# sony/timbre-trap

Measured on AMD Instinct MI355X. Metric: audio-seconds/s training throughput (9oct x 60bpo, 3s@22.05kHz), higher is better.
Workload: dtype bf16; 1 GPU; full train step (CQT x2 + AE fwd/bwd with consistency + 3 losses + clip + AdamW), model_complexity=2 latent=128, 64 clips x 3 s per GPU, under torch.autocast like reference experiments/train.py:415 (bf16 MFMA conv path of BASELINE config[2]; fp32 master weights, losses and optimizer); global_batch=64, parallelism=dp1

## Files before the change

### timbre-trap_amd/csrc/conv_edge_bf16.hip

```cpp
#include "bf16_common.h"
#include <type_traits>

namespace {

constexpr int ETH = 16, ETW = 64, ERW = ETW + 2, EROWS = ETH + 2;
constexpr int EPLANE = EROWS * ERW;
constexpr int PP = ETW + 8, PPLANE = EROWS * PP, PCOL0 = 3;
constexpr int NPARTW = 80;

__device__ __forceinline__ float gatef(float dy, float y) { return dy * elu_dout(y); }

struct ETile { int b, h0, t0; };
__device__ __forceinline__ ETile etile(int v, int tiles_h, int tiles_t, int ntiles) {
    int tile = xcd_order(v, ntiles);
    ETile r;
    r.t0 = (tile % tiles_t) * ETW; tile /= tiles_t;
    r.h0 = (tile % tiles_h) * ETH;
    r.b = tile / tiles_h;
    return r;
}

struct TileCtx { ETile tl; bool interior, interior_v; };
__device__ __forceinline__ TileCtx tile_ctx(int v, int tiles_h, int tiles_t, int ntiles, int H, int T) {
    TileCtx c;
// ... 428 lines not shown
        const ETile tl = etile(v, tiles_h, tiles_t, ntiles);
        __syncthreads();
        sx.store(xs, tid);
        __syncthreads();
        flush();
        if (v + gridDim.x < ntiles) sx.load(x, nullptr, tile_ctx(v + gridDim.x, tiles_h, tiles_t, ntiles, H, T), H, T, tid);
        PWin xw;
        xw.start(xs, r0, lane);
#pragma unroll
        for (int rr = 0; rr < ERPW; ++rr) {
            xw.advance(xs, r0 + rr, lane);
            if constexpr (NO == 2) {
                f32x2 a4[4] = {br, splat2(0.f), splat2(0.f), splat2(0.f)};
                static_for<0, 36>([&](auto ic) {
                    constexpr int ci = decltype(ic)::value / 9, k = decltype(ic)::value % 9;
                    a4[ci] = wr[ci * 9 + k] * xw.template tap<k, ci>() + a4[ci];
                });
                o[rr] = (a4[0] + a4[1]) + (a4[2] + a4[3]);
            } else {
                f32x2 a2[2] = {br, splat2(0.f)};
                static_for<0, 18>([&](auto ic) {
                    constexpr int p = decltype(ic)::value / 9, k = decltype(ic)::value % 9;
                    a2[p] = wr[p * 9 + k] * xw.template pair<k, p>() + a2[p];
                });
                const f32x2 a = a2[0] + a2[1];
                o[rr][0] = act_out(a[0] + a[1], ACT);
                o[rr][1] = 0.f;
            }
            asm volatile("" : "+v"(o[rr]));
            row_fence();
        }
        tp = tl;
    }
    flush();
}

template <bool VEC, int NO = 2, int ACT = TT_ACT_NONE>
__global__ __launch_bounds__(NT, 2) void k_cout_bwd(const e16* __restrict__ x, const float* __restrict__ dy, const float* __restrict__ w,
                                                  e16* __restrict__ dx, float* __restrict__ part, int H, int T, int tiles_h,
                                                  int tiles_t, int ntiles, float scale, const float* __restrict__ ysaved = nullptr) {
    constexpr int NW = NO * 36;
    __shared__ __attribute__((aligned(16))) float xs[4 * EPLANE + 4];
    __shared__ __attribute__((aligned(16))) float gs[NO * PPLANE];
    __shared__ float red[4 * (NW + NO)];
    const int tid = threadIdx.x, lane = tid & 63, wave = tid >> 6;
    float wa[NO * 9];
#pragma unroll
    for (int i = 0; i < NO * 9; ++i) wa[i] = scale * w[((i / 9) * 4 + (lane & 3)) * 9 + i % 9];
    f32x2 acc[NO == 2 ? 36 : 18], accb = splat2(0.f);
#pragma unroll
    for (int i = 0; i < (NO == 2 ? 36 : 18); ++i) acc[i] = splat2(0.f);
    StageCl4<false> sx;
    StagePlanar<NO, VEC, NO == 2 ? TT_ACT_NONE : ACT> sg;
    sx.init(T, tid); sg.init(H, T, tid);
    if (blockIdx.x < ntiles) {
        const TileCtx t0 = tile_ctx(blockIdx.x, tiles_h, tiles_t, ntiles, H, T);
        sx.load(x, nullptr, t0, H, T, tid); sg.load(dy, t0, H, T, tid, ysaved);
    }
    for (int v = blockIdx.x; v < ntiles; v += gridDim.x) {
        const ETile tl = etile(v, tiles_h, tiles_t, ntiles);
        __syncthreads();
        sx.store(xs, tid);
        sg.store(gs, tid);
        __syncthreads();
        if (v + gridDim.x < ntiles) {
            const TileCtx tn = tile_ctx(v + gridDim.x, tiles_h, tiles_t, ntiles, H, T);
            sx.load(x, nullptr, tn, H, T, tid); sg.load(dy, tn, H, T, tid, ysaved);
        }
        const int t = tl.t0 + lane, r0 = wave * ERPW;
        {
            PWin xw;
            xw.start(xs, r0, lane);
#pragma unroll
            for (int rr = 0; rr < ERPW; ++rr) {
                const int r = r0 + rr, ctr = (r + 1) * PP + lane + PCOL0 + 1;
                xw.advance(xs, r, lane);
                f32x2 g;
                if constexpr (NO == 2) {
                    g[0] = gs[ctr]; g[1] = gs[PPLANE + ctr];
                    accb += g;
                    static_for<0, 36>([&](auto ic) {
                        constexpr int i = decltype(ic)::value;
                        acc[i] = g * xw.template tap<i % 9, i / 9>() + acc[i];
                    });
                } else {
                    g = splat2(gs[ctr]);
                    accb[0] += g[0];
                    static_for<0, 18>([&](auto ic) {
                        constexpr int i = decltype(ic)::value;
                        acc[i] = g * xw.template pair<i % 9, i / 9>() + acc[i];
                    });
                }
                pin(acc); asm volatile("" : "+v"(accb));
                row_fence();
            }
        }
        f32x4 d[ERPW];
#pragma unroll
        for (int rr = 0; rr < ERPW; ++rr) d[rr] = f32x4{0.f, 0.f, 0.f, 0.f};
#pragma unroll
        for (int co = 0; co < NO; ++co) {
            WRow<1> gw[ERPW + 2];
#pragma unroll
            for (int i = 0; i < ERPW + 2; ++i) gw[i].load(gs + co * PPLANE, (r0 + i) * PP + lane + PCOL0);
            taps9<0>([&](auto kc) {
                constexpr int k = decltype(kc)::value;
#pragma unroll
                for (int rr = 0; rr < ERPW; ++rr) d[rr] = mfma441(wa[co * 9 + k], gw[rr + 2 - k / 3].template one<2 - k % 3>(0), d[rr]);
            });
            row_fence();
        }
#pragma unroll
        for (int rr = 0; rr < ERPW; ++rr) {
            const int h = tl.h0 + r0 + rr;
            e16x4 o;
            o[0] = (e16)d[rr][0]; o[1] = (e16)d[rr][1]; o[2] = (e16)d[rr][2]; o[3] = (e16)d[rr][3];
            if (t < T && h < H) *reinterpret_cast<e16x4*>(dx + (((long)tl.b * H + h) * T + t) * 4) = o;
        }
    }
    __syncthreads();
    float flat[NW + NO];
    if constexpr (NO == 2) {
#pragma unroll
        for (int i = 0; i < 36; ++i) { flat[i] = acc[i][0]; flat[36 + i] = acc[i][1]; }
        flat[72] = accb[0]; flat[73] = accb[1];
    } else {
#pragma unroll
        for (int i = 0; i < 18; ++i) { flat[(2 * (i / 9)) * 9 + i % 9] = acc[i][0]; flat[(2 * (i / 9) + 1) * 9 + i % 9] = acc[i][1]; }
        flat[36] = accb[0];
    }
    const float tot = wg_total<NW + NO>(flat, red, tid);
    if (tid < NW + NO) part[(long)blockIdx.x * NPARTW + tid] = tot;
}

__global__ __launch_bounds__(1024) void k_edge_reduce(const float* __restrict__ part, int nwg, float* __restrict__ dw, float* __restrict__ db,
                                                       int nb, float scale, int nw = 72) {
    __shared__ float red[16][64];
    const int el = threadIdx.x & 63, sl = threadIdx.x >> 6;
    const int e = blockIdx.x * 64 + el;
    float s = 0.f;
    if (e < nw + nb)
        for (int j = sl; j < nwg; j += 16) s += part[(long)j * NPARTW + e];
    red[sl][el] = s;
    __syncthreads();
    if (sl != 0 || e >= nw + nb) return;
    float sum = 0.f;
#pragma unroll
    for (int i = 0; i < 16; ++i) sum += red[i][el];
    if (e < nw) dw[e] += sum * scale; else db[e - nw] += sum * scale;
}

constexpr int EDGE_MAX_WG = 1024;

inline bool edge_ok(int B, int H, int T) { return B > 0 && H > 0 && T > 0 && (long)H * T * 4 < (1l << 31); }
inline void edge_tiles(int B, int H, int T, int& th, int& tt, int& n) { th = (H + ETH - 1) / ETH; tt = (T + ETW - 1) / ETW; n = B * th * tt; }
inline int edge_grid(int ntiles) { const int cap = 4 * tt_cus(); const int g = ntiles < cap ? ntiles : cap; return g < EDGE_MAX_WG ? g : EDGE_MAX_WG; }

}

extern "C" {

int64_t tt_edge16_scratch_bytes(void) { return (int64_t)EDGE_MAX_WG * NPARTW * 4; }

int tt_convin16_fwd(const float* x, const float* w, const float* b, void* y, int B, int H, int T, void* stream) {
    if (!x || !w || !b || !y || !edge_ok(B, H, T)) return TT_E_BADARG;
    int th, tt, n; edge_tiles(B, H, T, th, tt, n);
    if (T % 4 == 0) hipLaunchKernelGGL(k_cin_fwd<true>, dim3(edge_grid(n)), dim3(NT), 0, tt_stream(stream), x, w, b, (e16*)y, H, T, th, tt, n);
    else hipLaunchKernelGGL(k_cin_fwd<false>, dim3(edge_grid(n)), dim3(NT), 0, tt_stream(stream), x, w, b, (e16*)y, H, T, th, tt, n);
    TT_LAUNCH_CHECK();
    return 0;
}

int tt_convin16_bwd(const float* x, const void* y, const void* dy, const float* w, float* dx, float* dw, float* db, void* ws, int B,
                    int H, int T, void* stream) {
    if (!x || !dy || !w || !dw || !db || !ws || !edge_ok(B, H, T)) return TT_E_BADARG;
    int th, tt, n; edge_tiles(B, H, T, th, tt, n);
    const int grid = edge_grid(n);
    hipStream_t st = tt_stream(stream);
    const bool vec = T % 4 == 0;
#define CIN_BWD(DX_, V_, P_) hipLaunchKernelGGL((k_cin_bwd<DX_, V_, P_>), dim3(grid), dim3(NT), 0, st, x, (const e16*)y, (const e16*)dy, w, dx, (float*)ws, H, T, th, tt, n, tt_loss_unscale())
    if (y) {
        if (dx) { if (vec) CIN_BWD(true, true, false); else CIN_BWD(true, false, false); }
        else { if (vec) CIN_BWD(false, true, false); else CIN_BWD(false, false, false); }
    } else {
        if (dx) { if (vec) CIN_BWD(true, true, true); else CIN_BWD(true, false, true); }
        else { if (vec) CIN_BWD(false, true, true); else CIN_BWD(false, false, true); }
    }
#undef CIN_BWD
    TT_LAUNCH_CHECK();
    hipLaunchKernelGGL(k_edge_reduce, dim3(2), dim3(1024), 0, st, (const float*)ws, grid, dw, db, 4, tt_loss_unscale());
    TT_LAUNCH_CHECK();
    return 0;
}

int tt_convout16_fwd(const void* x, const float* w, const float* b, float* y, int B, int H, int T, void* stream) {
    if (!x || !w || !b || !y || !edge_ok(B, H, T)) return TT_E_BADARG;
    int th, tt, n; edge_tiles(B, H, T, th, tt, n);
    hipLaunchKernelGGL(k_cout_fwd, dim3(edge_grid(n)), dim3(NT), 0, tt_stream(stream), (const e16*)x, w, b, y, H, T, th, tt, n);
    TT_LAUNCH_CHECK();
    return 0;
}

int tt_convout16_bwd(const void* x, const float* dy, const float* w, void* dx, float* dw, float* db, void* ws, int B, int H, int T,
                     void* stream) {
    if (!x || !dy || !w || !dx || !dw || !db || !ws || !edge_ok(B, H, T)) return TT_E_BADARG;
    int th, tt, n; edge_tiles(B, H, T, th, tt, n);
    const int grid = edge_grid(n);
    hipStream_t st = tt_stream(stream);
    if (T % 4 == 0) hipLaunchKernelGGL(k_cout_bwd<true>, dim3(grid), dim3(NT), 0, st, (const e16*)x, dy, w, (e16*)dx, (float*)ws, H, T, th, tt, n, tt_loss_scale());
    else hipLaunchKernelGGL(k_cout_bwd<false>, dim3(grid), dim3(NT), 0, st, (const e16*)x, dy, w, (e16*)dx, (float*)ws, H, T, th, tt, n, tt_loss_scale());
    TT_LAUNCH_CHECK();
    hipLaunchKernelGGL(k_edge_reduce, dim3(2), dim3(1024), 0, st, (const float*)ws, grid, dw, db, 2, 1.f);
    TT_LAUNCH_CHECK();
    return 0;
}

int tt_convin16_1_fwd(const float* x, const float* w, const float* b, void* y, int B, int H, int T, void* stream) {
    if (!x || !w || !b || !y || !edge_ok(B, H, T)) return TT_E_BADARG;
    int th, tt, n; edge_tiles(B, H, T, th, tt, n);
    if (T % 4 == 0) hipLaunchKernelGGL((k_cin_fwd<true, 1>), dim3(edge_grid(n)), dim3(NT), 0, tt_stream(stream), x, w, b, (e16*)y, H, T, th, tt, n);
    else hipLaunchKernelGGL((k_cin_fwd<false, 1>), dim3(edge_grid(n)), dim3(NT), 0, tt_stream(stream), x, w, b, (e16*)y, H, T, th, tt, n);
    TT_LAUNCH_CHECK();
    return 0;
}

int tt_convin16_1_bwd(const float* x, const void* y, const void* dy, const float* w, float* dx, float* dw, float* db, void* ws, int B,
                      int H, int T, void* stream) {
    if (!x || !dy || !w || !dw || !db || !ws || !edge_ok(B, H, T)) return TT_E_BADARG;
    int th, tt, n; edge_tiles(B, H, T, th, tt, n);
    const int grid = edge_grid(n);
    hipStream_t st = tt_stream(stream);
    const bool vec = T % 4 == 0;
#define CIN1_BWD(DX_, V_, P_) hipLaunchKernelGGL((k_cin_bwd<DX_, V_, P_, 1>), dim3(grid), dim3(NT), 0, st, x, (const e16*)y, (const e16*)dy, w, dx, (float*)ws, H, T, th, tt, n, tt_loss_unscale())
    if (y) {
        if (dx) { if (vec) CIN1_BWD(true, true, false); else CIN1_BWD(true, false, false); }
        else { if (vec) CIN1_BWD(false, true, false); else CIN1_BWD(false, false, false); }
    } else {
        if (dx) { if (vec) CIN1_BWD(true, true, true); else CIN1_BWD(true, false, true); }
        else { if (vec) CIN1_BWD(false, true, true); else CIN1_BWD(false, false, true); }
    }
#undef CIN1_BWD
    TT_LAUNCH_CHECK();
    hipLaunchKernelGGL(k_edge_reduce, dim3(1), dim3(1024), 0, st, (const float*)ws, grid, dw, db, 4, tt_loss_unscale(), 36);
    TT_LAUNCH_CHECK();
    return 0;
}

int tt_convout16_1_fwd(const void* x, const float* w, const float* b, float* y, int B, int H, int T, int act, void* stream) {
    if (!x || !w || !b || !y || !edge_ok(B, H, T)) return TT_E_BADARG;
    int th, tt, n; edge_tiles(B, H, T, th, tt, n);
    hipStream_t st = tt_stream(stream);
    const dim3 grid(edge_grid(n));
    if (act == TT_ACT_NONE) hipLaunchKernelGGL((k_cout_fwd<1, TT_ACT_NONE>), grid, dim3(NT), 0, st, (const e16*)x, w, b, y, H, T, th, tt, n);
    else if (act == TT_ACT_RELU) hipLaunchKernelGGL((k_cout_fwd<1, TT_ACT_RELU>), grid, dim3(NT), 0, st, (const e16*)x, w, b, y, H, T, th, tt, n);
    else if (act == TT_ACT_SIGMOID) hipLaunchKernelGGL((k_cout_fwd<1, TT_ACT_SIGMOID>), grid, dim3(NT), 0, st, (const e16*)x, w, b, y, H, T, th, tt, n);
    else return TT_E_BADARG;
    TT_LAUNCH_CHECK();
    return 0;
}

int tt_convout16_1_bwd(const void* x, const float* y, const float* dy, const float* w, void* dx, float* dw, float* db, void* ws, int B, int H,
                       int T, int act, void* stream) {
    if (!x || !dy || !w || !dx || !dw || !db || !ws || !edge_ok(B, H, T)) return TT_E_BADARG;
    if ((act != TT_ACT_NONE && act != TT_ACT_RELU && act != TT_ACT_SIGMOID) || (act != TT_ACT_NONE && !y)) return TT_E_BADARG;
    int th, tt, n; edge_tiles(B, H, T, th, tt, n);
    const int grid = edge_grid(n);
    hipStream_t st = tt_stream(stream);
    const float s = tt_loss_scale();
#define COUT1_BWD(V_, A_) hipLaunchKernelGGL((k_cout_bwd<V_, 1, A_>), dim3(grid), dim3(NT), 0, st, (const e16*)x, dy, w, (e16*)dx, (float*)ws, H, T, th, tt, n, s, y)
    if (T % 4 == 0) {
        if (act == TT_ACT_NONE) COUT1_BWD(true, TT_ACT_NONE); else if (act == TT_ACT_RELU) COUT1_BWD(true, TT_ACT_RELU); else COUT1_BWD(true, TT_ACT_SIGMOID);
    } else {
        if (act == TT_ACT_NONE) COUT1_BWD(false, TT_ACT_NONE); else if (act == TT_ACT_RELU) COUT1_BWD(false, TT_ACT_RELU); else COUT1_BWD(false, TT_ACT_SIGMOID);
    }
#undef COUT1_BWD
    TT_LAUNCH_CHECK();
    hipLaunchKernelGGL(k_edge_reduce, dim3(1), dim3(1024), 0, st, (const float*)ws, grid, dw, db, 1, 1.f, 36);
    TT_LAUNCH_CHECK();
    return 0;
}

}
```

### timbre-trap_amd/timbre_trap/_hip.py

```python

import ctypes
import os
import subprocess
import sys

_HERE = os.path.dirname(os.path.abspath(__file__))
PKG_ROOT = os.path.dirname(_HERE)
REPO_ROOT = os.path.dirname(PKG_ROOT)
CSRC = os.path.join(PKG_ROOT, 'csrc')
LIB_PATH = os.path.join(PKG_ROOT, 'lib', 'libttrap_hip.so')
if os.environ.get('TTRAP_LIB'):
    LIB_PATH = os.path.join(PKG_ROOT, 'lib', os.environ['TTRAP_LIB'])
SOURCES = ['cqt.hip', 'cqt_generic.hip', 'conv_generic.hip', 'conv_mfma.hip', 'conv_small.hip', 'conv_wide_bf16.hip', 'conv_level_bf16.hip', 'conv_stride_bf16.hip',
           'latent_bf16.hip', 'conv_edge_bf16.hip', 'gemm.hip', 'losses.hip', 'magnitude.hip',
           'conv_wide_f16.hip', 'conv_level_f16.hip', 'conv_stride_f16.hip', 'latent_f16.hip', 'conv_edge_f16.hip',
           'conv_x3.hip',
           'sdr.hip',
           'mpe.hip',
           'resample.hip',
           'notes.hip',
           'pitch.hip',
           'film.hip',
           'mix.hip']

# ... 31 lines not shown
    'tt_conv2d_wgrad': (c_int, [P, P, P, P, I, I, I, I, I, I, I, I, I, I, I, I, I, L, L, L, L, P]),
    'tt_elu_bwd': (c_int, [P, P, P, L, P]),
    'tt_act_bwd': (c_int, [P, P, P, L, I, P]),
    'tt_cqt_forward_mag': (c_int, [ctypes.POINTER(CqtPlan), P, P, P, I, I, P]),
    'tt_magnitude': (c_int, [P, P, L, L, P]),
    'tt_decibels_scratch_bytes': (c_int64, [L]),
    'tt_decibels': (c_int, [P, P, L, L, I, P, P]),
    'tt_activations1_fwd': (c_int, [P, P, L, P]),
    'tt_activations1_bwd': (c_int, [P, P, P, L, P]),
    'tt_resblock_fwd': (c_int, [P, P, P, P, P, P, P, I, I, I, I, I, I, P]),
    'tt_resblock_bwd': (c_int, [P, P, P, P, P, P, P, P, P, P, P, P, P, I, I, I, I, I, I, P]),
    'tt_wide_scratch_bytes': (c_int64, [I, I, I, I]),
    'tt_wide_pack': (c_int, [P, P, I, I, I, I, P]),
    'tt_wide_unpack': (c_int, [P, P, I, I, I, I, P]),
    'tt_wide_rb_fwd': (c_int, [P, P, P, P, P, P, P, I, I, I, I, I, P]),
    'tt_wide_rb_fwd_join': (c_int, [P, P, P, P, P, P, P, P, P, I, I, I, I, I, I, I, P]),
    'tt_wide_rb_bwd': (c_int, [P, P, P, P, P, P, P, P, P, P, P, P, I, I, I, I, I, P]),
    'tt_wide_level_scratch_bytes': (c_int64, [I, I, I, I, I]),
    'tt_wide_level_bwd': (c_int, [I, P, P, P, P, P, P, P, P, P, P, P, P, P, P, I, I, I, I, P, P]),
    'tt_wide_level_bwd_gated': (c_int, [I, P, P, P, P, P, P, P, P, P, P, P, P, P, P, I, I, I, I, P, P]),
    'tt_wide_level_bwd_gated_join': (c_int, [I, P, P, P, P, P, P, P, P, P, P, P, P, P, P, I, I, I, I, P, P, I, P, I, P, P]),
    'tt_x3_bytes': (c_int64, [I, I, I, I]),
    'tt_x3_level_scratch_bytes': (c_int64, [I, I, I, I]),
    'tt_x3_pack': (c_int, [P, P, I, I, I, I, P]),
    'tt_x3_unpack': (c_int, [P, P, I, I, I, I, P]),
    'tt_x3_rb_fwd': (c_int, [P, P, P, P, P, P, I, I, I, I, I, I, P]),
    'tt_x3_level_fwd': (c_int, [I, P, I, P, I, P, P, P, P, P, P, I, I, I, I, P]),
    'tt_x3_rb_fwd_train': (c_int, [P, P, P, P, P, P, I, P, I, I, I, I, I, P]),
    'tt_x3_grad_scale_scratch_bytes': (c_int64, []),
    'tt_x3_grad_scale': (c_int, [P, c_int64, P, P, P]),
    'tt_x3_pack_scaled': (c_int, [P, P, P, I, I, I, I, P]),
    'tt_x3_unpack_scaled': (c_int, [P, P, P, I, I, I, I, P]),
    'tt_x3_rb_bwd_scratch_bytes': (c_int64, [I, I, I, I]),
    'tt_x3_rb_bwd': (c_int, [P, P, P, P, P, P, P, I, P, P, P, P, P, P, I, I, I, I, I, P]),
    'tt_x3n_level_scratch_bytes': (c_int64, [I, I, I, I]),
    'tt_x3n_rb_fwd': (c_int, [P, I, P, P, P, P, P, I, I, I, I, I, I, P]),
    'tt_x3n_level_fwd': (c_int, [I, P, P, P, P, P, P, P, P, I, I, I, I, P]),
    'tt_x3_latent_scratch_bytes': (c_int64, [I, I, I]),
    'tt_x3_latent_encode': (c_int, [P, P, P, P, P, I, I, I, I, I, P]),
    'tt_x3_latent_decode': (c_int, [P, I, c_float, P, P, P, I, P, I, I, I, I, I, P]),
    'tt_x3_sconv_fwd': (c_int, [P, I, P, P, P, I, I, I, I, I, P]),
    'tt_x3_tconv_fwd': (c_int, [P, I, P, P, P, I, I, I, I, I, I, P]),
    'tt_wide_fused_scratch_bytes': (c_int64, [I]),
    'tt_wide_rb_bwd_fused': (c_int, [P, P, P, P, P, P, P, P, P, P, P, P, I, I, I, I, I, P]),
    'tt_wide_onepass_scratch_bytes': (c_int64, [I]),
    'tt_wide_rb_bwd_onepass': (c_int, [P, P, P, P, P, P, P, P, P, P, P, P, I, I, I, I, I, P]),
    'tt_wide_rb_bwd_is_onepass': (c_int, [I, I]),
    'tt_wide_bwd_kernel_attr': (c_int, [I, I, I, I, ctypes.POINTER(c_int), ctypes.POINTER(c_int)]),
    'tt_stride16_scratch_bytes': (c_int64, [I]),
    'tt_sconv16_fwd': (c_int, [P, P, P, P, I, I, I, I, P]),
    'tt_sconv16_bwd': (c_int, [P, P, P, P, P, P, P, P, I, I, I, I, P]),
    'tt_tconv16_fwd': (c_int, [P, P, P, P, I, I, I, I, I, P]),
    'tt_tconv16_bwd': (c_int, [P, P, P, P, P, P, P, P, I, I, I, I, I, P]),
    'tt_gate16': (c_int, [P, P, L, P]),
    'tt_sconv16_bwd_pregated': (c_int, [P, P, P, P, P, P, P, I, I, I, I, P]),
    'tt_tconv16_bwd_pregated': (c_int, [P, P, P, P, P, P, P, I, I, I, I, I, I, P]),
    'tt_latent16_pregated_ok': (c_int, [I, I]),
    'tt_latent16_expand_gated': (c_int, [P, P, P, P, P, I, I, I, I, I, P]),
    'tt_latent16_contract_pregated': (c_int, [P, P, P, P, I, I, I, I, I, I, P]),
    'tt_latent16_wgrad_pregated': (c_int, [P, I, F_, P, P, P, P, I, I, I, I, I, P]),
    'tt_latent16_scratch_bytes': (c_int64, [I, I, I, I, I]),
    'tt_latent16_contract': (c_int, [P, P, P, P, P, P, I, I, I, I, I, I, P]),
    'tt_latent16_expand': (c_int, [P, I, F_, P, P, P, P, I, I, I, I, I, P]),
    'tt_latent16_wgrad': (c_int, [P, I, F_, P, P, P, P, P, I, I, I, I, I, P]),
    'tt_edge16_scratch_bytes': (c_int64, []),
    'tt_convin16_fwd': (c_int, [P, P, P, P, I, I, I, P]),
    'tt_convin16_bwd': (c_int, [P, P, P, P, P, P, P, P, I, I, I, P]),
    'tt_convout16_fwd': (c_int, [P, P, P, P, I, I, I, P]),
    'tt_convout16_bwd': (c_int, [P, P, P, P, P, P, P, I, I, I, P]),
    'tt_convin16_1_fwd': (c_int, [P, P, P, P, I, I, I, P]),
    'tt_convin16_1_bwd': (c_int, [P, P, P, P, P, P, P, P, I, I, I, P]),
    'tt_convout16_1_fwd': (c_int, [P, P, P, P, I, I, I, I, P]),
    'tt_convout16_1_bwd': (c_int, [P, P, P, P, P, P, P, P, I, I, I, I, P]),
    'tt_sconv_fwd': (c_int, [P, P, P, P, I, I, I, I, P]),
    'tt_wgrad_scratch_floats': (c_int64, []),
    'tt_sconv_bwd': (c_int, [P, P, P, P, P, P, P, P, I, I, I, I, P]),
    'tt_tconv_fwd': (c_int, [P, P, P, P, I, I, I, I, I, P]),
    'tt_tconv_bwd': (c_int, [P, P, P, P, P, P, P, P, I, I, I, I, I, P]),
    'tt_gemm': (c_int, [P, P, P, P, I, I, I, I, I, L, L, L, I, L, L, L, I, F_, F_, I, I, I, P]),
    'tt_channel_sum': (c_int, [P, P, I, I, L, P]),
    'tt_channel_sum_ws': (c_int, [P, P, I, I, L, P, P]),
    'tt_scaled_add': (c_int, [P, P, P, I, P, L, P]),
    'tt_window_ola': (c_int, [P, P, P, L, I, I, I, L, P]),
    'tt_dot': (c_int, [P, P, P, L, P]),
    'tt_scaled_add16': (c_int, [P, P, P, I, P, L, P]),
    'tt_dot16': (c_int, [P, P, P, L, P]),
    'tt_skip_join16_fwd': (c_int, [P, P, P, I, P, L, I, P]),
    'tt_skip_join16_bwd': (c_int, [P, P, P, I, P, P, L, I, I, P]),
    'tt_sqdiff_sum': (c_int, [P, P, P, P, L, F_, P]),
    'tt_sqdiff_bwd': (c_int, [P, P, P, F_, P, P, L, P]),
    'tt_sqdiff2_bwd': (c_int, [P, P, P, P, P, F_, P, P, P, L, P]),
    'tt_sqdiff_sum_grad': (c_int, [P, P, P, P, L, F_, P, P, P]),
    'tt_sqdiff2_sum_grad': (c_int, [P, P, P, P, P, P, L, F_, P, P, P, P]),
    'tt_sqdiff_rescale': (c_int, [P, P, P, L, P]),
    'tt_sqdiff2_rescale': (c_int, [P, P, P, P, P, L, P]),
    'tt_activations_fwd': (c_int, [P, P, I, I, I, P]),
    'tt_activations_bwd': (c_int, [P, P, P, P, I, I, I, P]),
    'tt_transcription_loss_fwd': (c_int, [P, P, P, P, P, I, I, I, I, P]),
    'tt_transcription_loss_fwd_grad': (c_int, [P, P, P, P, P, P, I, I, I, I, P]),
    'tt_transcription_loss_bwd': (c_int, [P, P, P, P, P, I, I, I, I, P]),
    'tt_segment_stats': (c_int, [P, P, I, P, P]),
    'tt_peak_pick': (c_int, [P, P, L, I, I, ctypes.c_double, I, I, P]),
    'tt_target_activations': (c_int, [P, P, I, P, I, I, I, P, P, P]),
    'tt_target_activations_spans': (c_int, [P, P, P, I, P, I, I, I, P, P, P]),
    'tt_sdr_chunk': (c_int, []),
    'tt_sdr_scratch_bytes': (c_int64, [I, L, I]),
    'tt_sdr_means': (c_int, [P, P, I, L, P, P, P]),
    'tt_sdr_correlate': (c_int, [P, P, I, L, I, P, P, P, P]),
    'tt_sdr_finish': (c_int, [P, I, I, ctypes.c_double, I, P, P, P]),
    'tt_mpe_max_est': (c_int, []),
    'tt_mpe_max_ref': (c_int, []),
    'tt_mpe_count': (c_int, [P, I, I, ctypes.c_double, I, I, P, P, P, P]),
    'tt_mpe_fill': (c_int, [P, I, I, ctypes.c_double, I, I, P, L, P, P]),
    'tt_mpe_match': (c_int, [P, I, I, P, P, P, I, P, P, ctypes.c_double, P, P, P, P]),
    'tt_note_tile_frames': (c_int, []),
    'tt_note_chunk': (c_int, []),
    'tt_note_spans': (c_int, [P, I, P, I, P, P, P]),
    'tt_note_count': (c_int, [P, P, I, I, P, P]),
    'tt_note_fill': (c_int, [P, P, I, I, P, L, P, P]),
    'tt_pitch_tile_frames': (c_int, []),
    'tt_pitch_max_bins': (c_int, []),
    'tt_pitch_max_radius': (c_int, []),
    'tt_pitch_scratch_bytes': (c_int64, [I, I]),
    'tt_pitch_nearest': (c_int, [P, P, I, P, P, I, I, P, P]),
    'tt_pitch_targets': (c_int, [P, P, I, P, I, I, P, P, P, P, I, I, I, P, P, P, P]),
    'tt_film_tile_frames': (c_int, []),
    'tt_film_scratch_bytes': (c_int64, [I, I, I, I]),
    'tt_film_fwd': (c_int, [P, P, P, P, P, P, P, I, I, I, I, P]),
    'tt_film_bwd': (c_int, [P, P, P, P, P, P, P, P, P, P, P, I, I, I, I, P]),
    'tt_mix_tile': (c_int, []),
    'tt_mix_targets_tile': (c_int, []),
    'tt_mix_audio': (c_int, [P, P, I, P, P, P, P, I, L, P, P]),
    'tt_mix_targets': (c_int, [P, P, I, I, L, I, P, P]),
    'tt_resample_tile': (c_int, []),
    'tt_resample_direct_tile': (c_int, []),
    'tt_resample_max_taps': (c_int, []),
    'tt_resample_max_phases': (c_int, []),
    'tt_resample_partials': (c_int64, [L, I, I]),
    'tt_resample': (c_int, [P, I, I, L, P, I, I, I, P, L, P, P]),
    'tt_resample_normalize': (c_int, [P, I, L, P, L, P]),
    'tt_l2norm': (c_int, [P, P, P, L, P]),
    'tt_adamw_step': (c_int, [P, P, P, P, P, L, F_, F_, F_, F_, F_, I, F_, I, P, P]),
    'tt_set_loss_scale': (c_float, [F_]),
}
HALF_TWINS = ('tt_wide_level_scratch_bytes', 'tt_wide_level_bwd', 'tt_wide_level_bwd_gated', 'tt_wide_level_bwd_gated_join', 'tt_gate16', 'tt_latent16_pregated_ok', 'tt_latent16_expand_gated', 'tt_latent16_contract_pregated', 'tt_latent16_wgrad_pregated', 'tt_sconv16_bwd_pregated', 'tt_tconv16_bwd_pregated', 'tt_wide_scratch_bytes', 'tt_wide_pack', 'tt_wide_unpack', 'tt_wide_rb_fwd', 'tt_wide_rb_fwd_join', 'tt_wide_rb_bwd', 'tt_wide_fused_scratch_bytes',
              'tt_wide_rb_bwd_fused', 'tt_wide_onepass_scratch_bytes', 'tt_wide_rb_bwd_onepass', 'tt_wide_rb_bwd_is_onepass', 'tt_wide_bwd_kernel_attr',
              'tt_stride16_scratch_bytes', 'tt_sconv16_fwd', 'tt_sconv16_bwd', 'tt_tconv16_fwd', 'tt_tconv16_bwd', 'tt_latent16_scratch_bytes',
              'tt_latent16_contract', 'tt_latent16_expand', 'tt_latent16_wgrad', 'tt_edge16_scratch_bytes', 'tt_convin16_fwd', 'tt_convin16_bwd',
              'tt_convout16_fwd', 'tt_convout16_bwd', 'tt_convin16_1_fwd', 'tt_convin16_1_bwd', 'tt_convout16_1_fwd', 'tt_convout16_1_bwd',
              'tt_scaled_add16', 'tt_dot16', 'tt_skip_join16_fwd', 'tt_skip_join16_bwd')
for _n in HALF_TWINS:
    _PROTOS[_n + '_h'] = _PROTOS[_n]
EXPORTED_SYMBOLS = tuple(_PROTOS)
EXTRA_FLAGS = {'cqt.hip': ['-fno-slp-vectorize']}


def build(verbose=False, force=False):
    srcs = [os.path.join(CSRC, s) for s in SOURCES]
    deps = srcs + [os.path.join(CSRC, 'common.h'), os.path.join(REPO_ROOT, 'include', 'ttrap.h')]
    deps += [os.path.join(CSRC, f) for f in os.listdir(CSRC) if f.endswith('.h')] + [os.path.abspath(__file__)]
    if os.environ.get('TTRAP_LIB'):
        if not os.path.exists(LIB_PATH):
            raise RuntimeError('TTRAP_LIB=%s: %s does not exist (build it with tools/build_variant.sh)' % (os.environ['TTRAP_LIB'], LIB_PATH))
        return LIB_PATH
    if not force and os.path.exists(LIB_PATH) and all(os.path.getmtime(LIB_PATH) >= os.path.getmtime(d) for d in deps):
        return LIB_PATH
    os.makedirs(os.path.dirname(LIB_PATH), exist_ok=True)
    hipcc = os.environ.get('HIPCC', '/opt/rocm/bin/hipcc')
    objs = []
    jobs = []
    for s in srcs:
        base = os.path.basename(s)
        o = os.path.join(PKG_ROOT, 'lib', base.replace('.hip', '.o'))
        objs.append(o)
        jobs.append([hipcc, '--offload-arch=gfx950', '-O3', '-std=c++17', '-fPIC'] + EXTRA_FLAGS.get(base, []) + ['-c', s, '-o', o])
    width = max(1, min(len(jobs), os.cpu_count() or 1))
    running, failed = [], None
    pending = list(jobs)
    while pending or running:
        while pending and len(running) < width:
            cmd = pending.pop(0)
            if verbose:
                print(' '.join(cmd), file=sys.stderr)
            running.append((cmd, subprocess.Popen(cmd, stdout=subprocess.PIPE, stderr=subprocess.STDOUT)))
        cmd, pr = running.pop(0)
        out, _ = pr.communicate()
        if pr.returncode != 0 and failed is None:
            failed = 'hipcc failed: %s\n%s' % (' '.join(cmd), out.decode())
            pending = []
    if failed:
        raise RuntimeError(failed)
    for f in os.listdir(os.path.dirname(LIB_PATH)):
        if f.endswith('.o') and os.path.join(os.path.dirname(LIB_PATH), f) not in objs:
            os.remove(os.path.join(os.path.dirname(LIB_PATH), f))
    tmp = LIB_PATH + '.tmp.%d' % os.getpid()
    cmd = [hipcc, '--offload-arch=gfx950', '-shared', '-fPIC', '-o', tmp] + objs
    subprocess.run(cmd, check=True)
    os.replace(tmp, LIB_PATH)
    return LIB_PATH


def lib():
    global _lib
    if _lib is None:
        if not os.path.exists(LIB_PATH):
            raise RuntimeError(
                'libttrap_hip.so not found at %s -- run `python -c "import __graft_entry__ as g; g.build()"` '
                '(there is no CPU fallback for the Timbre-Trap HIP path)' % LIB_PATH)
        import torch
        h = ctypes.CDLL(LIB_PATH)
        for name, (res, args) in _PROTOS.items():
            fn = getattr(h, name)
            fn.restype = res
            fn.argtypes = args
        _lib = h
    return _lib


def check(rc, what=''):
    if rc != 0:
        msg = lib().tt_error_string(rc)
        raise RuntimeError('ttrap HIP call %s failed (%d): %s' % (what, rc, msg.decode() if msg else '?'))


EVENT_LOG = None
EVENT_KEYS = None


class timed:

    def __init__(self, key, clips=None):
        self.key = key
        self.clips = clips
        self.start = None

    def __enter__(self):
        if EVENT_LOG is not None and (EVENT_KEYS is None or self.key in EVENT_KEYS):
            import torch
            self.start = torch.cuda.Event(enable_timing=True)
            self.start.record()
        return self

    def __exit__(self, *exc):
        if self.start is not None:
            import torch
            end = torch.cuda.Event(enable_timing=True)
            end.record()
            EVENT_LOG.setdefault(self.key, []).append((self.start, end, self.clips))
        return False


def stream_ptr():
    import torch
    return ctypes.c_void_p(torch.cuda.current_stream().cuda_stream)


def ptr(t):
    return None if t is None else ctypes.c_void_p(t.data_ptr())


def require_cuda(*tensors):
    for t in tensors:
        if t is not None and not t.is_cuda:
            raise RuntimeError('timbre_trap HIP path needs tensors on the GPU (got %s); there is no CPU fallback'
                               % t.device)
```

Baseline: 3982 audio-seconds/s.

## Replace edge conv forward tiles with per-wave strip-walking kernels using DPP shifts

```diff
diff --git a/timbre-trap_amd/csrc/conv_edge_bf16.hip b/timbre-trap_amd/csrc/conv_edge_bf16.hip
--- a/timbre-trap_amd/csrc/conv_edge_bf16.hip
+++ b/timbre-trap_amd/csrc/conv_edge_bf16.hip
@@ -604,6 +604,16 @@
 
 constexpr int EDGE_MAX_WG = 1024;
 
+#include "conv_edge_strip.h"
+
+inline int strip_grid_fwd(const SGeom& g) { return (g.units + 3) / 4; }
+inline int strip_grid_bwd(const SGeom& g) {
+    const int n = (g.units + 3) / 4, cap = TT_EDGE_OCC_B * tt_cus() < EDGE_MAX_WG ? TT_EDGE_OCC_B * tt_cus() : EDGE_MAX_WG;
+    return n < cap ? n : cap;
+}
+
+inline bool strip_bwd() { return tt_switch("TTRAP_EDGE_STRIP_BWD", 0) != 0; }
+
 inline bool edge_ok(int B, int H, int T) { return B > 0 && H > 0 && T > 0 && (long)H * T * 4 < (1l << 31); }
 inline void edge_tiles(int B, int H, int T, int& th, int& tt, int& n) { th = (H + ETH - 1) / ETH; tt = (T + ETW - 1) / ETW; n = B * th * tt; }
 inline int edge_grid(int ntiles) { const int cap = 4 * tt_cus(); const int g = ntiles < cap ? ntiles : cap; return g < EDGE_MAX_WG ? g : EDGE_MAX_WG; }
@@ -616,9 +626,8 @@
 
 int tt_convin16_fwd(const float* x, const float* w, const float* b, void* y, int B, int H, int T, void* stream) {
     if (!x || !w || !b || !y || !edge_ok(B, H, T)) return TT_E_BADARG;
-    int th, tt, n; edge_tiles(B, H, T, th, tt, n);
-    if (T % 4 == 0) hipLaunchKernelGGL(k_cin_fwd<true>, dim3(edge_grid(n)), dim3(NT), 0, tt_stream(stream), x, w, b, (e16*)y, H, T, th, tt, n);
-    else hipLaunchKernelGGL(k_cin_fwd<false>, dim3(edge_grid(n)), dim3(NT), 0, tt_stream(stream), x, w, b, (e16*)y, H, T, th, tt, n);
+    const SGeom g = strip_geom(B, H, T, TT_EDGE_WPC_F, TT_EDGE_RF);
+    hipLaunchKernelGGL(k_es_cin_fwd, dim3(strip_grid_fwd(g)), dim3(NT), 0, tt_stream(stream), x, w, b, (e16*)y, H, T, g);
     TT_LAUNCH_CHECK();
     return 0;
 }
@@ -626,19 +635,29 @@
 int tt_convin16_bwd(const float* x, const void* y, const void* dy, const float* w, float* dx, float* dw, float* db, void* ws, int B,
                     int H, int T, void* stream) {
     if (!x || !dy || !w || !dw || !db || !ws || !edge_ok(B, H, T)) return TT_E_BADARG;
-    int th, tt, n; edge_tiles(B, H, T, th, tt, n);
-    const int grid = edge_grid(n);
     hipStream_t st = tt_stream(stream);
-    const bool vec = T % 4 == 0;
+    int grid;
+    if (strip_bwd()) {
+        const SGeom g = strip_geom(B, H, T, TT_EDGE_WPC_B, TT_EDGE_RB);
+        grid = strip_grid_bwd(g);
+#define CIN_BWD(DX_, P_) hipLaunchKernelGGL((k_es_cin_bwd<DX_, P_>), dim3(grid), dim3(NT), 0, st, x, (const e16*)y, (const e16*)dy, w, dx, (float*)ws, H, T, g, tt_loss_unscale())
+        if (y) { if (dx) CIN_BWD(true, false); else CIN_BWD(false, false); }
+        else { if (dx) CIN_BWD(true, true); else CIN_BWD(false, true); }
+#undef CIN_BWD
+    } else {
+        int th, tt, n; edge_tiles(B, H, T, th, tt, n);
+        grid = edge_grid(n);
+        const bool vec = T % 4 == 0;
 #define CIN_BWD(DX_, V_, P_) hipLaunchKernelGGL((k_cin_bwd<DX_, V_, P_>), dim3(grid), dim3(NT), 0, st, x, (const e16*)y, (const e16*)dy, w, dx, (float*)ws, H, T, th, tt, n, tt_loss_unscale())
-    if (y) {
-        if (dx) { if (vec) CIN_BWD(true, true, false); else CIN_BWD(true, false, false); }
-        else { if (vec) CIN_BWD(false, true, false); else CIN_BWD(false, false, false); }
-    } else {
-        if (dx) { if (vec) CIN_BWD(true, true, true); else CIN_BWD(true, false, true); }
-        else { if (vec) CIN_BWD(false, true, true); else CIN_BWD(false, false, true); }
-    }
+        if (y) {
+            if (dx) { if (vec) CIN_BWD(true, true, false); else CIN_BWD(true, false, false); }
+            else { if (vec) CIN_BWD(false, true, false); else CIN_BWD(false, false, false); }
+        } else {
+            if (dx) { if (vec) CIN_BWD(true, true, true); else CIN_BWD(true, false, true); }
+            else { if (vec) CIN_BWD(false, true, true); else CIN_BWD(false, false, true); }
+        }
 #undef CIN_BWD
+    }
     TT_LAUNCH_CHECK();
     hipLaunchKernelGGL(k_edge_reduce, dim3(2), dim3(1024), 0, st, (const float*)ws, grid, dw, db, 4, tt_loss_unscale());
     TT_LAUNCH_CHECK();
@@ -647,8 +666,8 @@
 
 int tt_convout16_fwd(const void* x, const float* w, const float* b, float* y, int B, int H, int T, void* stream) {
     if (!x || !w || !b || !y || !edge_ok(B, H, T)) return TT_E_BADARG;
-    int th, tt, n; edge_tiles(B, H, T, th, tt, n);
-    hipLaunchKernelGGL(k_cout_fwd, dim3(edge_grid(n)), dim3(NT), 0, tt_stream(stream), (const e16*)x, w, b, y, H, T, th, tt, n);
+    const SGeom g = strip_geom(B, H, T, TT_EDGE_WPC_F, TT_EDGE_RF);
+    hipLaunchKernelGGL(k_es_cout_fwd, dim3(strip_grid_fwd(g)), dim3(NT), 0, tt_stream(stream), (const e16*)x, w, b, y, H, T, g);
     TT_LAUNCH_CHECK();
     return 0;
 }
@@ -656,11 +675,18 @@
 int tt_convout16_bwd(const void* x, const float* dy, const float* w, void* dx, float* dw, float* db, void* ws, int B, int H, int T,
                      void* stream) {
     if (!x || !dy || !w || !dx || !dw || !db || !ws || !edge_ok(B, H, T)) return TT_E_BADARG;
-    int th, tt, n; edge_tiles(B, H, T, th, tt, n);
-    const int grid = edge_grid(n);
     hipStream_t st = tt_stream(stream);
-    if (T % 4 == 0) hipLaunchKernelGGL(k_cout_bwd<true>, dim3(grid), dim3(NT), 0, st, (const e16*)x, dy, w, (e16*)dx, (float*)ws, H, T, th, tt, n, tt_loss_scale());
-    else hipLaunchKernelGGL(k_cout_bwd<false>, dim3(grid), dim3(NT), 0, st, (const e16*)x, dy, w, (e16*)dx, (float*)ws, H, T, th, tt, n, tt_loss_scale());
+    int grid;
+    if (strip_bwd()) {
+        const SGeom g = strip_geom(B, H, T, TT_EDGE_WPC_B, TT_EDGE_RB);
+        grid = strip_grid_bwd(g);
+        hipLaunchKernelGGL(k_es_cout_bwd, dim3(grid), dim3(NT), 0, st, (const e16*)x, dy, w, (e16*)dx, (float*)ws, H, T, g, tt_loss_scale());
+    } else {
+        int th, tt, n; edge_tiles(B, H, T, th, tt, n);
+        grid = edge_grid(n);
+        if (T % 4 == 0) hipLaunchKernelGGL(k_cout_bwd<true>, dim3(grid), dim3(NT), 0, st, (const e16*)x, dy, w, (e16*)dx, (float*)ws, H, T, th, tt, n, tt_loss_scale());
+        else hipLaunchKernelGGL(k_cout_bwd<false>, dim3(grid), dim3(NT), 0, st, (const e16*)x, dy, w, (e16*)dx, (float*)ws, H, T, th, tt, n, tt_loss_scale());
+    }
     TT_LAUNCH_CHECK();
     hipLaunchKernelGGL(k_edge_reduce, dim3(2), dim3(1024), 0, st, (const float*)ws, grid, dw, db, 2, 1.f);
     TT_LAUNCH_CHECK();
diff --git a/timbre-trap_amd/csrc/conv_edge_strip.h b/timbre-trap_amd/csrc/conv_edge_strip.h
--- /dev/null
+++ b/timbre-trap_amd/csrc/conv_edge_strip.h
@@ -0,0 +1,356 @@
+#pragma once
+
+#ifndef TT_EDGE_RF
+#define TT_EDGE_RF 9
+#endif
+#ifndef TT_EDGE_RB
+#define TT_EDGE_RB 3
+#endif
+#ifndef TT_EDGE_OCC_B
+#define TT_EDGE_OCC_B 3
+#endif
+#ifndef TT_EDGE_WPC_F
+#define TT_EDGE_WPC_F 32
+#endif
+#ifndef TT_EDGE_WPC_B
+#define TT_EDGE_WPC_B 24
+#endif
+
+constexpr int SW = 62;
+constexpr int SEG_FLOOR = 8;
+static_assert(TT_EDGE_RF % 3 == 0 && TT_EDGE_RB % 3 == 0, "ring depth: a multiple of the window's three rows");
+
+typedef unsigned u32x2 __attribute__((ext_vector_type(2)));
+
+struct SGeom { int strips, nseg, seglen, units; };
+struct SUnit { int b, t0, h0, h1; };
+__device__ __forceinline__ SUnit sunit(int u, const SGeom& g, int H) {
+    SUnit r;
+    r.t0 = (u % g.strips) * SW; u /= g.strips;
+    r.h0 = (u % g.nseg) * g.seglen;
+    r.b = u / g.nseg;
+    r.h1 = r.h0 + g.seglen < H ? r.h0 + g.seglen : H;
+    return r;
+}
+struct SLane {
+    unsigned tc, tp;
+    bool col, own, ownp;
+    __device__ __forceinline__ void set(int t0, int T, int lane) {
+        const int tl = t0 + lane - 1;
+        col = tl >= 0 && tl < T;
+        tc = (unsigned)(tl < 0 ? 0 : tl < T ? tl : T - 1);
+        own = col && lane >= 1 && lane <= 62;
+        ownp = lane >= 2 && tl - 1 < T;
+        tp = ownp ? (unsigned)(tl - 1) : 0u;
+    }
+};
+template <bool LEFT> __device__ __forceinline__ float sshift(float v) {
+    return __builtin_bit_cast(float, __builtin_amdgcn_update_dpp(0, __builtin_bit_cast(int, v), LEFT ? 0x138 : 0x130, 0xf, 0xf, true));
+}
+__device__ __forceinline__ u32x2 smask(u32x2 v, bool ok) { v[0] = ok ? v[0] : 0u; v[1] = ok ? v[1] : 0u; return v; }
+__device__ __forceinline__ f32x4 sfloat4(u32x2 raw) {
+    const e16x4 q = __builtin_bit_cast(e16x4, raw);
+    return f32x4{(float)q[0], (float)q[1], (float)q[2], (float)q[3]};
+}
+__device__ __forceinline__ u32x2 spack4(f32x4 v) {
+    e16x4 o;
+    o[0] = (e16)v[0]; o[1] = (e16)v[1]; o[2] = (e16)v[2]; o[3] = (e16)v[3];
+    return __builtin_bit_cast(u32x2, o);
+}
+typedef __amdgpu_buffer_rsrc_t srsrc;
+__device__ __forceinline__ srsrc sres(const void* p, unsigned bytes) {
+    return __builtin_amdgcn_make_buffer_rsrc(const_cast<void*>(p), 0, (int)bytes, 0x00020000);
+}
+__device__ __forceinline__ u32x2 sload_cl(srsrc r, int row, int T, const SLane& ln) {
+    return __builtin_amdgcn_raw_buffer_load_b64(r, ln.tc * 8u, (unsigned)row * (unsigned)T * 8u, 0);
+}
+__device__ __forceinline__ void sstore_cl(srsrc r, int row, int T, const SLane& ln, u32x2 v) {
+    __builtin_amdgcn_raw_buffer_store_b64(v, r, ln.tc * 8u, (unsigned)row * (unsigned)T * 8u, 0);
+}
+struct RawPl { float a, b; };
+__device__ __forceinline__ RawPl sload_pl(srsrc r, int row, int H, int T, const SLane& ln) {
+    RawPl v;
+    v.a = __builtin_bit_cast(float, __builtin_amdgcn_raw_buffer_load_b32(r, ln.tc * 4u, (unsigned)row * (unsigned)T * 4u, 0));
+    v.b = __builtin_bit_cast(float, __builtin_amdgcn_raw_buffer_load_b32(r, ln.tc * 4u, (unsigned)(H + row) * (unsigned)T * 4u, 0));
+    return v;
+}
+__device__ __forceinline__ void sstore_pl(srsrc r, int row, int H, int T, const SLane& ln, float a, float b) {
+    __builtin_amdgcn_raw_buffer_store_b32(__builtin_bit_cast(unsigned, a), r, ln.tc * 4u, (unsigned)row * (unsigned)T * 4u, 0);
+    __builtin_amdgcn_raw_buffer_store_b32(__builtin_bit_cast(unsigned, b), r, ln.tc * 4u, (unsigned)(H + row) * (unsigned)T * 4u, 0);
+}
+__device__ __forceinline__ void sstore_pl_prev(srsrc r, int row, int H, int T, const SLane& ln, float a, float b) {
+    __builtin_amdgcn_raw_buffer_store_b32(__builtin_bit_cast(unsigned, a), r, ln.tp * 4u, (unsigned)row * (unsigned)T * 4u, 0);
+    __builtin_amdgcn_raw_buffer_store_b32(__builtin_bit_cast(unsigned, b), r, ln.tp * 4u, (unsigned)(H + row) * (unsigned)T * 4u, 0);
+}
+__device__ __forceinline__ int sclamp(int r, int hi) { return r < 0 ? 0 : r < hi ? r : hi; }
+
+template <int R, class I, class S, class C>
+__device__ __forceinline__ void strip_walk(int h0, int h1, I&& issue, S&& take, C&& compute) {
+    static_for<0, R>([&](auto ic) { issue(ic, h0 + decltype(ic)::value); });
+    for (int q = h0; q < h1; q += R)
+        static_for<0, R>([&](auto ic) {
+            constexpr int i = decltype(ic)::value;
+            take(ic, q + i);
+            issue(ic, q + i + R);
+            compute(ic, q + i, q + i < h1);
+            row_fence();
+        });
+}
+__device__ __forceinline__ int strip_wave() { return blockIdx.x * 4 + __builtin_amdgcn_readfirstlane(threadIdx.x >> 6); }
+
+template <int N> struct SRow { float c[3][N]; };
+template <int N> __device__ __forceinline__ void sfill(SRow<N>& w, const float (&ctr)[N]) {
+#pragma unroll
+    for (int i = 0; i < N; ++i) { w.c[1][i] = ctr[i]; w.c[0][i] = sshift<true>(ctr[i]); w.c[2][i] = sshift<false>(ctr[i]); }
+}
+__global__ __launch_bounds__(NT, 4) void k_es_cout_fwd(const e16* __restrict__ x, const float* __restrict__ w, const float* __restrict__ bias,
+                                                       float* __restrict__ y, int H, int T, SGeom g) {
+    constexpr int R = TT_EDGE_RF;
+    const int lane = threadIdx.x & 63, nwv = gridDim.x * 4;
+    constexpr int NSW = 24;
+    float wr[72];
+#pragma unroll
+    for (int i = 0; i < 72; ++i) { wr[i] = w[i]; if (i >= NSW) asm volatile("" : "+v"(wr[i])); }
+    const float b0 = bias[0], b1 = bias[1];
+    for (int u = strip_wave(); u < g.units; u += nwv) {
+        const SUnit un = sunit(u, g, H);
+        SLane ln; ln.set(un.t0, T, lane);
+        const unsigned clip = (unsigned)H * (unsigned)T * 8u;
+        const srsrc xb = sres(x + (long)un.b * H * T * 4, clip), yb = sres(y + (long)un.b * 2 * H * T, clip);
+        SRow<4> win[3];
+        u32x2 ring[R];
+        auto fill = [&](SRow<4>& wrow, u32x2 raw, int row) {
+            const f32x4 v = sfloat4(smask(raw, ln.col && row >= 0 && row < H));
+            const float ctr[4] = {v[0], v[1], v[2], v[3]};
+            sfill<4>(wrow, ctr);
+        };
+        fill(win[1], sload_cl(xb, sclamp(un.h0 - 1, H - 1), T, ln), un.h0 - 1);
+        fill(win[2], sload_cl(xb, un.h0, T, ln), un.h0);
+        strip_walk<R>(un.h0, un.h1,
+            [&](auto ic, int q) { ring[decltype(ic)::value] = sload_cl(xb, sclamp(q + 1 < un.h1 ? q + 1 : un.h1, H - 1), T, ln); },
+            [&](auto ic, int q) { constexpr int i = decltype(ic)::value; fill(win[i % 3], ring[i], q + 1); },
+            [&](auto ic, int q, bool live) {
+                constexpr int i = decltype(ic)::value;
+                float a[4] = {b0, 0.f, 0.f, 0.f}, c[4] = {b1, 0.f, 0.f, 0.f};
+                static_for<0, 36>([&](auto jc) {
+                    constexpr int ci = decltype(jc)::value / 9, k = decltype(jc)::value % 9;
+                    const float xv = win[(i + 1 + k / 3) % 3].c[k % 3][ci];
+                    a[ci] = __builtin_fmaf(wr[ci * 9 + k], xv, a[ci]);
+                    c[ci] = __builtin_fmaf(wr[36 + ci * 9 + k], xv, c[ci]);
+                });
+                if (ln.own && live) sstore_pl(yb, q, H, T, ln, (a[0] + a[1]) + (a[2] + a[3]), (c[0] + c[1]) + (c[2] + c[3]));
+            });
+    }
+}
+
+__global__ __launch_bounds__(NT, 4) void k_es_cin_fwd(const float* __restrict__ x, const float* __restrict__ w, const float* __restrict__ bias,
+                                                      e16* __restrict__ y, int H, int T, SGeom g) {
+    constexpr int R = TT_EDGE_RF;
+    const int lane = threadIdx.x & 63, nwv = gridDim.x * 4;
+    float wa[18];
+#pragma unroll
+    for (int i = 0; i < 18; ++i) wa[i] = w[(lane & 3) * 18 + i];
+    const f32x4 br = {bias[0], bias[1], bias[2], bias[3]};
+    for (int u = strip_wave(); u < g.units; u += nwv) {
+        const SUnit un = sunit(u, g, H);
+        SLane ln; ln.set(un.t0, T, lane);
+        const unsigned clip = (unsigned)H * (unsigned)T * 8u;
+        const srsrc xb = sres(x + (long)un.b * 2 * H * T, clip), yb = sres(y + (long)un.b * H * T * 4, clip);
+        SRow<2> win[3];
+        RawPl ring[R];
+        auto fill = [&](SRow<2>& wrow, const RawPl& rw, int row) {
+            const bool ok = ln.col && row >= 0 && row < H;
+            const float ctr[2] = {ok ? rw.a : 0.f, ok ? rw.b : 0.f};
+            sfill<2>(wrow, ctr);
+        };
+        fill(win[1], sload_pl(xb, sclamp(un.h0 - 1, H - 1), H, T, ln), un.h0 - 1);
+        fill(win[2], sload_pl(xb, un.h0, H, T, ln), un.h0);
+        strip_walk<R>(un.h0, un.h1,
+            [&](auto ic, int q) { ring[decltype(ic)::value] = sload_pl(xb, sclamp(q + 1 < un.h1 ? q + 1 : un.h1, H - 1), H, T, ln); },
+            [&](auto ic, int q) { constexpr int i = decltype(ic)::value; fill(win[i % 3], ring[i], q + 1); },
+            [&](auto ic, int q, bool live) {
+                constexpr int i = decltype(ic)::value;
+                f32x4 a0 = br, a1 = {0.f, 0.f, 0.f, 0.f};
+                static_for<0, 9>([&](auto kc) {
+                    constexpr int k = decltype(kc)::value;
+                    a0 = mfma441(wa[k], win[(i + 1 + k / 3) % 3].c[k % 3][0], a0);
+                    a1 = mfma441(wa[9 + k], win[(i + 1 + k / 3) % 3].c[k % 3][1], a1);
+                });
+                const f32x4 a = a0 + a1;
+                const f32x4 o = {elu_f(a[0]), elu_f(a[1]), elu_f(a[2]), elu_f(a[3])};
+                if (ln.own && live) sstore_cl(yb, q, T, ln, spack4(o));
+            });
+    }
+}
+
+template <int N> __device__ __forceinline__ void strip_partials(float (&flat)[N], float* red, float* part) {
+    const float tot = wg_total<N>(flat, red, threadIdx.x);
+    if (threadIdx.x < N) part[(long)blockIdx.x * NPARTW + threadIdx.x] = tot;
+}
+
+__global__ __launch_bounds__(NT, TT_EDGE_OCC_B) void k_es_cout_bwd(const e16* __restrict__ x, const float* __restrict__ dy, const float* __restrict__ w,
+                                                       e16* __restrict__ dx, float* __restrict__ part, int H, int T, SGeom g, float scale) {
+    constexpr int R = TT_EDGE_RB;
+    __shared__ float red[4 * 74];
+    const int lane = threadIdx.x & 63, nwv = gridDim.x * 4;
+    float wa[18];
+#pragma unroll
+    for (int i = 0; i < 18; ++i) wa[i] = scale * w[((i / 9) * 4 + (lane & 3)) * 9 + i % 9];
+    float acc[72], accb[2] = {0.f, 0.f};
+#pragma unroll
+    for (int i = 0; i < 72; ++i) acc[i] = 0.f;
+    struct Slot { u32x2 xq; RawPl g; };
+    for (int u = strip_wave(); u < g.units; u += nwv) {
+        const SUnit un = sunit(u, g, H);
+        SLane ln; ln.set(un.t0, T, lane);
+        const unsigned clip = (unsigned)H * (unsigned)T * 8u;
+        const srsrc xb = sres(x + (long)un.b * H * T * 4, clip), gb = sres(dy + (long)un.b * 2 * H * T, clip);
+        const srsrc db_ = sres(dx + (long)un.b * H * T * 4, clip);
+        SRow<2> win[3];
+        Slot ring[R];
+        f32x4 xv;
+        auto fill = [&](SRow<2>& wrow, const RawPl& rw, int row) {
+            const bool ok = ln.col && row >= 0 && row < H;
+            const float ctr[2] = {ok ? rw.a : 0.f, ok ? rw.b : 0.f};
+            sfill<2>(wrow, ctr);
+        };
+        fill(win[1], sload_pl(gb, sclamp(un.h0 - 1, H - 1), H, T, ln), un.h0 - 1);
+        fill(win[2], sload_pl(gb, un.h0, H, T, ln), un.h0);
+        strip_walk<R>(un.h0, un.h1,
+            [&](auto ic, int q) {
+                constexpr int i = decltype(ic)::value;
+                const int qc = q < un.h1 ? q : un.h1 - 1;
+                ring[i].xq = sload_cl(xb, qc, T, ln);
+                ring[i].g = sload_pl(gb, sclamp(qc + 1, H - 1), H, T, ln);
+            },
+            [&](auto ic, int q) {
+                constexpr int i = decltype(ic)::value;
+                xv = sfloat4(smask(ring[i].xq, ln.own && q < un.h1));
+                fill(win[i % 3], ring[i].g, q + 1);
+            },
+            [&](auto ic, int q, bool live) {
+                constexpr int i = decltype(ic)::value;
+                const float lv = live ? 1.f : 0.f;
+                accb[0] = __builtin_fmaf(win[(i + 2) % 3].c[1][0], lv, accb[0]); accb[1] = __builtin_fmaf(win[(i + 2) % 3].c[1][1], lv, accb[1]);
+                f32x4 d = {0.f, 0.f, 0.f, 0.f};
+                static_for<0, 18>([&](auto jc) {
+                    constexpr int co = decltype(jc)::value / 9, k = decltype(jc)::value % 9;
+                    const float gv = win[(i + 1 + (2 - k / 3)) % 3].c[2 - k % 3][co];
+#pragma unroll
+                    for (int ci = 0; ci < 4; ++ci) acc[(co * 4 + ci) * 9 + k] = __builtin_fmaf(xv[ci], gv, acc[(co * 4 + ci) * 9 + k]);
+                    d = mfma441(wa[co * 9 + k], gv, d);
+                });
+                if (ln.own && live) sstore_cl(db_, q, T, ln, spack4(d));
+            });
+    }
+    float flat[74];
+#pragma unroll
+    for (int i = 0; i < 72; ++i) flat[i] = acc[i];
+    const bool counts = lane >= 1 && lane <= 62;
+    flat[72] = counts ? accb[0] : 0.f; flat[73] = counts ? accb[1] : 0.f;
+    strip_partials<74>(flat, red, part);
+}
+
+template <bool DX, bool PRE>
+__global__ __launch_bounds__(NT, TT_EDGE_OCC_B) void k_es_cin_bwd(const float* __restrict__ x, const e16* __restrict__ y, const e16* __restrict__ dy,
+                                                      const float* __restrict__ w, float* __restrict__ dx, float* __restrict__ part, int H, int T,
+                                                      SGeom g, float unscale) {
+    constexpr int R = TT_EDGE_RB;
+    __shared__ float red[4 * 76];
+    const int lane = threadIdx.x & 63, nwv = gridDim.x * 4;
+    constexpr int NSW = 48;
+    float wr[DX ? 72 : 1];
+    if constexpr (DX) {
+#pragma unroll
+        for (int i = 0; i < 72; ++i) { wr[i] = w[i]; if (i >= NSW) asm volatile("" : "+v"(wr[i])); }
+    }
+    float acc[72], accb[4] = {0.f, 0.f, 0.f, 0.f};
+#pragma unroll
+    for (int i = 0; i < 72; ++i) acc[i] = 0.f;
+    struct Slot { RawPl x; u32x2 g, yy; };
+    for (int u = strip_wave(); u < g.units; u += nwv) {
+        const SUnit un = sunit(u, g, H);
+        SLane ln; ln.set(un.t0, T, lane);
+        const unsigned clip = (unsigned)H * (unsigned)T * 8u;
+        const srsrc xb = sres(x + (long)un.b * 2 * H * T, clip), gb = sres(dy + (long)un.b * H * T * 4, clip);
+        const srsrc yb = sres(PRE ? dy : y + (long)un.b * H * T * 4, clip), db_ = sres(DX ? dx + (long)un.b * 2 * H * T : nullptr, clip);
+        float gc[3][4];
+        Slot ring[R];
+        float xs[3][2];
+        auto fill = [&](float (&row4)[4], u32x2 rg, u32x2 ry, int row) {
+            const bool ok = ln.col && row >= 0 && row < H;
+            if constexpr (PRE) { const f32x4 v = sfloat4(smask(rg, ok)); for (int c = 0; c < 4; ++c) row4[c] = v[c]; }
+            else { const f32x4 v = sfloat4(rg), yv = sfloat4(ry); for (int c = 0; c < 4; ++c) row4[c] = ok ? gatef(v[c], yv[c]) : 0.f; }
+        };
+        auto ldy = [&](int row) { return PRE ? u32x2{0u, 0u} : sload_cl(yb, row, T, ln); };
+        {
+            const int r0 = sclamp(un.h0 - 1, H - 1);
+            fill(gc[1], sload_cl(gb, r0, T, ln), ldy(r0), un.h0 - 1);
+            fill(gc[2], sload_cl(gb, un.h0, T, ln), ldy(un.h0), un.h0);
+        }
+        strip_walk<R>(un.h0, un.h1,
+            [&](auto ic, int q) {
+                constexpr int i = decltype(ic)::value;
+                const int qc = q < un.h1 ? q : un.h1 - 1, rn = sclamp(qc + 1, H - 1);
+                ring[i].x = sload_pl(xb, qc, H, T, ln);
+                ring[i].g = sload_cl(gb, rn, T, ln);
+                ring[i].yy = ldy(rn);
+            },
+            [&](auto ic, int q) {
+                constexpr int i = decltype(ic)::value;
+                const bool xok = ln.own && q < un.h1;
+                const float xv[2] = {xok ? ring[i].x.a : 0.f, xok ? ring[i].x.b : 0.f};
+#pragma unroll
+                for (int ci = 0; ci < 2; ++ci) { xs[1][ci] = xv[ci]; xs[0][ci] = sshift<true>(xv[ci]); xs[2][ci] = sshift<false>(xv[ci]); }
+                fill(gc[i % 3], ring[i].g, ring[i].yy, q + 1);
+            },
+            [&](auto ic, int q, bool live) {
+                constexpr int i = decltype(ic)::value;
+                const float lv = live ? 1.f : 0.f;
+#pragma unroll
+                for (int co = 0; co < 4; ++co) accb[co] = __builtin_fmaf(gc[(i + 2) % 3][co], lv, accb[co]);
+                static_for<0, 36>([&](auto jc) {
+                    constexpr int co = decltype(jc)::value / 9, k = decltype(jc)::value % 9, kh = k / 3, kw = k % 3;
+                    const float gv = gc[(i + 1 + (2 - kh)) % 3][co];
+#pragma unroll
+                    for (int ci = 0; ci < 2; ++ci) acc[(co * 2 + ci) * 9 + k] = __builtin_fmaf(gv, xs[kw][ci], acc[(co * 2 + ci) * 9 + k]);
+                });
+                if constexpr (DX) {
+                    float d[2] = {0.f, 0.f};
+                    static_for<0, 3>([&](auto jc) {
+                        constexpr int kw = 2 - decltype(jc)::value;
+                        static_for<0, 12>([&](auto qc) {
+                            constexpr int co = decltype(qc)::value / 3, kh = decltype(qc)::value % 3;
+                            const float gv = gc[(i + 1 + (2 - kh)) % 3][co];
+#pragma unroll
+                            for (int ci = 0; ci < 2; ++ci) d[ci] = __builtin_fmaf(wr[(co * 2 + ci) * 9 + kh * 3 + kw], gv, d[ci]);
+                        });
+                        if constexpr (kw > 0) { d[0] = sshift<true>(d[0]); d[1] = sshift<true>(d[1]); }
+                    });
+                    if (ln.ownp && live) sstore_pl_prev(db_, q, H, T, ln, d[0] * unscale, d[1] * unscale);
+                }
+            });
+    }
+    float flat[76];
+#pragma unroll
+    for (int i = 0; i < 72; ++i) flat[i] = acc[i];
+    const bool counts = lane >= 1 && lane <= 62;
+#pragma unroll
+    for (int co = 0; co < 4; ++co) flat[72 + co] = counts ? accb[co] : 0.f;
+    strip_partials<76>(flat, red, part);
+}
+
+inline SGeom strip_geom(int B, int H, int T, int wpc, int R) {
+    SGeom g;
+    g.strips = (T + SW - 1) / SW;
+    const long cols = (long)B * g.strips, want = (long)wpc * tt_cus();
+    long nseg = (want + cols - 1) / cols;
+    if (nseg < 1) nseg = 1;
+    int len = (int)((H + nseg - 1) / nseg);
+    if (len < SEG_FLOOR) len = SEG_FLOOR;
+    len = (len + R - 1) / R * R;
+    g.seglen = len;
+    g.nseg = (H + len - 1) / len;
+    g.units = (int)(cols * g.nseg);
+    return g;
+}
diff --git a/timbre-trap_amd/timbre_trap/_hip.py b/timbre-trap_amd/timbre_trap/_hip.py
--- a/timbre-trap_amd/timbre_trap/_hip.py
+++ b/timbre-trap_amd/timbre_trap/_hip.py
@@ -207,7 +207,7 @@
 for _n in HALF_TWINS:
     _PROTOS[_n + '_h'] = _PROTOS[_n]
 EXPORTED_SYMBOLS = tuple(_PROTOS)
-EXTRA_FLAGS = {'cqt.hip': ['-fno-slp-vectorize']}
+EXTRA_FLAGS = {'cqt.hip': ['-fno-slp-vectorize'], 'conv_edge_bf16.hip': ['-fno-slp-vectorize'], 'conv_edge_f16.hip': ['-fno-slp-vectorize']}
 
 
 def build(verbose=False, force=False):
```

After: 3957 audio-seconds/s. No clear change (-0.6%).
